# hpc4cmb/flacarray

Hardware: AMD Instinct MI355X
Metric: Msamples/s encode+decode, 4096ch x 1Msamp int32 (higher is better)
Workload: dtype int32

## Files before the change

### flacarray_amd/csrc/encode_fused.hpp

```cpp
#pragma once
#include "encode_kernels.hpp"
#include "quantize_kernels.hpp"

namespace fa {

constexpr int kFSmpWords = 65 * 32;
#ifndef FA_F_SCANW
#define FA_F_SCANW 4
#endif
#ifndef FA_F_RING
#define FA_F_RING 1024
#endif
constexpr int kFRingWords = FA_F_RING;
constexpr int kFRingMask = kFRingWords - 1;
constexpr int kFRingBlocks = kFRingWords / 64;
constexpr int kFRowBlocks = 12;
static_assert(kFRingBlocks - kFRowBlocks - 1 >= 1, "the ring must hold the longest row and a partial block beside what waits to be flushed");
constexpr int kFWaveWords = kFSmpWords + kFRingWords + 4 + 16;
constexpr int kFWaves = 4;
constexpr int kFCrcSlice = 1024;
constexpr int kFCrcXpow = 520;
#ifndef FA_F_SLEEP
#define FA_F_SLEEP 8
#endif
// ... 31 lines not shown
    const float* win;
    const uint4* hdr;
    uint8_t* blob;
    int64_t capacity;
    int64_t hb;
    uint32_t* frame_bytes;
    int64_t* frame_abs;
    FrameInfo* info;
    uint32_t* ticket;
    uint32_t* size_pub;
    unsigned long long* off_pub;
    int64_t* total;
    int* err;
    const uint16_t* crc_tab;
    unsigned long long* stamps;
    int64_t* starts;
    int64_t* nbytes;
};

__device__ __forceinline__ int fsmp_unit(int c1, int u) { return 32 * c1 + 4 * (u ^ (c1 & 7)); }
__device__ __forceinline__ int fsmp_idx(int s) {
    const int c1 = (s >> 5) + 1;
    return fsmp_unit(c1, (s >> 2) & 7) + (s & 3);
}

__device__ __forceinline__ int lane_id_opaque() {
    int l;
    asm volatile("v_mbcnt_lo_u32_b32 %0, -1, 0\n\tv_mbcnt_hi_u32_b32 %0, -1, %0" : "=v"(l));
    return l;
}
__device__ __forceinline__ int rice_fold(int r) { return (int)(((uint32_t)r << 1) ^ (uint32_t)(r >> 31)); }
__device__ __forceinline__ int dpp_wave_shr1(int old, int v) { return __builtin_amdgcn_update_dpp(old, v, 0x138, 0xF, 0xF, false); }

__device__ __forceinline__ uint16_t crc16_mulmod(uint16_t a, uint16_t b) {
    uint32_t r = 0;
#pragma unroll
    for (int i = 15; i >= 0; --i) {
        r = (r << 1) ^ ((r & 0x8000u) ? 0x18005u : 0u);
        if ((b >> i) & 1) r ^= a;
    }
    return (uint16_t)r;
}

template <typename T>
__device__ __forceinline__ T lb_load(const T* p) { return __hip_atomic_load(p, __ATOMIC_RELAXED, __HIP_MEMORY_SCOPE_AGENT); }

struct SplitRiceSearch {
    int pred_order, pmax, lane;
    uint32_t TA, TB, S, n, pb, SC, best;
    int M, p, k, bpo, kb;
    bool slot;
    __device__ __forceinline__ void start(uint32_t ta, uint32_t tb, int pred_order_, int pmax_, int lane_) {
        pred_order = pred_order_; pmax = pmax_; lane = lane_;
        TA = wave_incl_scan_u32(ta);
        TB = wave_incl_scan_u32(tb);
    }
    __device__ __forceinline__ void gather() {
        M = (2 << pmax) - 1;
        const int Lp = M - lane;
        slot = (Lp >= 1);
        const int po = slot ? (31 - __clz(Lp)) : 0;
        p = lane - (M + 1 - (2 << po));
        const uint32_t psz = 4096u >> po;
        const int cpp = 128 >> po;
        const bool inB = (po > 0) && (p >= (1 << (po - 1)));
        const int ph = inB ? (p - (1 << (po - 1))) : p;
        int hi_l = (po == 0) ? 63 : ((ph + 1) * cpp - 1);
        int lo_l = (po == 0) ? -1 : (ph * cpp - 1);
        hi_l &= 63;
        const int lo_c = lo_l < 0 ? 0 : (lo_l & 63);
        const uint32_t ah = (uint32_t)__builtin_amdgcn_ds_bpermute(hi_l << 2, (int)TA);
        const uint32_t bh = (uint32_t)__builtin_amdgcn_ds_bpermute(hi_l << 2, (int)TB);
        const uint32_t al = (uint32_t)__builtin_amdgcn_ds_bpermute(lo_c << 2, (int)TA);
        const uint32_t bl = (uint32_t)__builtin_amdgcn_ds_bpermute(lo_c << 2, (int)TB);
        uint32_t s;
        if (po == 0) s = ah + bh;
        else s = (inB ? bh : ah) - ((lo_l >= 0) ? (inB ? bl : al) : 0u);
        S = slot ? s : 0u;
        n = psz - ((p == 0) ? (uint32_t)pred_order : 0u);
        n = slot ? n : 1u;
    }
    __device__ __forceinline__ void params() {
        const uint32_t fpd = 0x40000u / n;
        const uint32_t m1 = S - 1;
        const uint32_t v = (__umulhi(m1, fpd) << 14) | ((m1 * fpd) >> 18);
        k = (S < 2 || v == 0) ? 0 : (32 - __clz((int)v));
        const uint32_t rest = (k != 0) ? (S >> ((k - 1) & 31)) : (S << 1);
        pb = 4u + (uint32_t)(1 + k) * n + rest - (n >> 1);
        pb = slot ? pb : 0u;
    }
    __device__ __forceinline__ void totals() {
        SC = wave_incl_scan_u32(pb);
        best = 0xffffffffu;
        bpo = 0;
        kb = 0;
    }
    __device__ __forceinline__ void order(int o) {
        const bool valid = (o <= pmax);
        const int base = valid ? (M + 1 - (2 << o)) : 0;
        const int end = valid ? (base + (1 << o) - 1) : 0;
        const uint32_t hi = (uint32_t)__builtin_amdgcn_readlane((int)SC, end);
        const uint32_t lo = (uint32_t)__builtin_amdgcn_readlane((int)SC, base > 0 ? base - 1 : 0);
        const uint32_t bits = hi - (base > 0 ? lo : 0u) + 6u;
        const int kg = __builtin_amdgcn_ds_bpermute(((base + lane) & 63) << 2, k);
        const bool take = valid && (bits < best);
        best = take ? bits : best;
        bpo = take ? o : bpo;
        kb = take ? kg : kb;
    }
};

__device__ __forceinline__ uint64_t split_rice_search_slow(uint64_t ta, uint64_t tb, int pred_order, int pmax, int lane, int* best_po,
                                                           int* kbest) {
    const uint64_t TA = wave_incl_scan_u64(ta), TB = wave_incl_scan_u64(tb);
    uint64_t best = 0;
    bool have = false;
// ... 59 lines not shown
                if ((uint32_t)lane < cnt) {
                    const uint64_t off = prefix + (incl - mine) + (uint64_t)(i / nf + 1u) * (uint64_t)a.hb;
                    __hip_atomic_store(a.off_pub + i, (unsigned long long)off, __ATOMIC_RELAXED, __HIP_MEMORY_SCOPE_AGENT);
#ifdef FA_TIMELINE
                    if (a.info) a.info[i].porder = (int32_t)(uint32_t)__builtin_amdgcn_s_memrealtime();
#endif
                }
                prefix += (uint32_t)__builtin_amdgcn_readlane((int)incl, 63);
                adv += cnt;
            }
            open = open && (cnt == 64u);
        }
        pos += adv;
        if (adv == 0) {
            __builtin_amdgcn_s_sleep(4);
            if (++idle > kLbSpinLimit) {
                if (lane == 0) atomicOr(a.err, 4);
                return;
            }
        } else {
            idle = 0;
        }
    }
    if (lane == 0) *a.total = (int64_t)(prefix + (uint64_t)a.n_stream * (uint64_t)a.hb);
}

#if defined(FA_UNIT_FUSED) || !defined(FA_SPLIT_UNITS)
template <int MLO, bool F32IN = false>
__global__ __launch_bounds__(256) __attribute__((amdgpu_waves_per_eu(MLO > 8 ? 2 : FA_F_WAVES, MLO > 8 ? 2 : FA_F_WAVES))) void encode_fused_kernel(FusedArgs a) {
    static_assert(MLO > 0, "levels 0-2 (fixed predictors, 1152-sample blocks) use the slot path");
    __shared__ __attribute__((aligned(16))) int32_t lds_all[kFWaves * kFWaveWords];
    __shared__ __attribute__((aligned(16))) uint16_t crc_s[kFCrcSlice];
    __shared__ uint32_t ticket_s;

    const int tid = threadIdx.x;
    const int lane = tid & 63;
    const int wave = __builtin_amdgcn_readfirstlane(tid >> 6);
    for (int i = tid; i < kFCrcSlice / 2; i += 256) reinterpret_cast<uint32_t*>(crc_s)[i] = reinterpret_cast<const uint32_t*>(a.crc_tab)[i];
    if (tid == 0) ticket_s = __hip_atomic_fetch_add(a.ticket, 1u, __ATOMIC_RELAXED, __HIP_MEMORY_SCOPE_AGENT);
    __syncthreads();
    const uint32_t ticket = (uint32_t)__builtin_amdgcn_readfirstlane((int)ticket_s);
    if (ticket == 0) {
        if (wave == 0) fused_scanner(a, lane);
        return;
    }
    const int64_t g = (int64_t)(ticket - 1) * kFWaves + wave;
    if (g >= a.total_frames) return;

    int32_t* smp = lds_all + wave * kFWaveWords;
    uint32_t* ring = reinterpret_cast<uint32_t*>(smp + kFSmpWords);
    uint8_t* kpar = reinterpret_cast<uint8_t*>(smp + kFSmpWords + kFRingWords + 4);
    uint32_t* scr = ring;

    const int64_t s = (int64_t)((uint32_t)g / (uint32_t)a.nframes);
    const int64_t f = g - s * a.nframes;
    if (f == a.nframes - 1 && a.tail_bs != kMaxBlock) return;
    constexpr int bs = kMaxBlock;
    const int32_t* src = a.data + (s * a.stream_size + f * (int64_t)bs);
    float q_off = 0.0f, q_gain = 0.0f;
    if constexpr (F32IN) { q_off = a.f_offsets[s]; q_gain = a.f_gains[s]; }
    auto load_row = [&](int j) __attribute__((always_inline)) {
        const int4 v = reinterpret_cast<const int4*>(src)[64 * j + lane];
        if constexpr (F32IN)
            return make_int4(quantise_f32(__int_as_float(v.x), q_off, q_gain), quantise_f32(__int_as_float(v.y), q_off, q_gain),
                             quantise_f32(__int_as_float(v.z), q_off, q_gain), quantise_f32(__int_as_float(v.w), q_off, q_gain));
        else
            return v;
    };
    const float* win = a.win;
    const uint4 fhe = a.hdr[f];
    const uint32_t fh_bits = 32u + ((fhe.w >> 8) & 0xFFu) + ((fhe.w >> 16) & 0xFFu) + (fhe.w >> 24) + 8u;

#define FA_IMAGE_ADDRS                                                                  \
    const int ln_ = lane_id_opaque();                                                   \
    const int K = fsmp_unit(ln_ + 1, 0);                                                \
    const int rowbase = fsmp_unit((ln_ >> 3) + 1, ln_ & 7);                             \
    const int hist7 = fsmp_unit(ln_, 7), hist6 = fsmp_unit(ln_, 6), hist5 = fsmp_unit(ln_, 5); \
    (void)K; (void)rowbase; (void)hist7; (void)hist6; (void)hist5
    constexpr int tailA7 = 32 * 64 + 4 * (7 ^ (64 & 7)), tailA6 = 32 * 64 + 4 * (6 ^ (64 & 7)), tailA5 = 32 * 64 + 4 * (5 ^ (64 & 7));

    FA_STAMP_INIT;
#ifdef FA_TIMELINE
    const uint32_t tl_start_ = (uint32_t)__builtin_amdgcn_s_memrealtime();
#endif
    int4 Bv[8];
    uint32_t orv = 0;
    int mn, mx;
    {
        FA_IMAGE_ADDRS;
        int4 hi[8], lo[8];
#pragma unroll
        for (int j = 0; j < 8; ++j) hi[j] = load_row(8 + j);
#pragma unroll
        for (int j = 0; j < 8; ++j) lo[j] = load_row(j);
        if (lane < 32) smp[lane] = 0;
        mn = hi[0].x;
        mx = hi[0].x;
#pragma unroll
        for (int j = 0; j < 8; ++j) {
            orv |= (uint32_t)(hi[j].x | hi[j].y | hi[j].z | hi[j].w);
            mn = min(min(mn, hi[j].x), hi[j].y);
            mn = min(min(mn, hi[j].z), hi[j].w);
            mx = max(max(mx, hi[j].x), hi[j].y);
            mx = max(max(mx, hi[j].z), hi[j].w);
            *reinterpret_cast<int4*>(&smp[rowbase + 256 * j]) = hi[j];
        }
#pragma unroll
        for (int t = 0; t < 8; ++t) Bv[t] = *reinterpret_cast<const int4*>(&smp[K ^ (4 * t)]);
#pragma unroll
        for (int j = 0; j < 8; ++j) {
            orv |= (uint32_t)(lo[j].x | lo[j].y | lo[j].z | lo[j].w);
            mn = min(min(mn, lo[j].x), lo[j].y);
            mn = min(min(mn, lo[j].z), lo[j].w);
            mx = max(max(mx, lo[j].x), lo[j].y);
            mx = max(max(mx, lo[j].z), lo[j].w);
            *reinterpret_cast<int4*>(&smp[rowbase + 256 * j]) = lo[j];
        }
    }
    mn = wave_min_i32(mn);
    mx = wave_max_i32(mx);
    const bool is_const = (mn == mx);
    orv = wave_or_u32(orv);
    const int wasted = orv ? (__ffs((int)orv) - 1) : 0;
    const int bps = 32 - wasted;
    if (__builtin_expect(wasted != 0, 0)) {
        FA_IMAGE_ADDRS;
#pragma unroll
        for (int t = 0; t < 8; ++t) {
            Bv[t].x >>= wasted; Bv[t].y >>= wasted; Bv[t].z >>= wasted; Bv[t].w >>= wasted;
            int4* p = reinterpret_cast<int4*>(&smp[K ^ (4 * t)]);
            int4 v = *p;
            v.x >>= wasted; v.y >>= wasted; v.z >>= wasted; v.w >>= wasted;
            *p = v;
        }
        mn >>= wasted;
        mx >>= wasted;
    }
    const bool narrow = (mn >= -(1 << 24)) && (mx < (1 << 24));
    lds_fence();

    FA_STAMP(0);
    const uint64_t verbatim_bits = 8 + (uint64_t)wasted + (uint64_t)bs * (uint64_t)bps;
    int type = 1;
    int order = 0, porder = 0, shift = 0, precision = 0;
    int kbest = 0;
    bool img_is_residual = false;
    bool win_small_l = false, win_small_f = false;
    int fo = -1;
    int32_t qkeep[MLO];
#pragma unroll
    for (int j = 0; j < MLO; ++j) qkeep[j] = 0;
    const int pmax_geo = a.pmax_full;
    auto pmax_for = [&](int pred_order) __attribute__((always_inline)) {
        int pm = pmax_geo;
        while (pm > 0 && (bs >> pm) <= pred_order) pm--;
        return pm;
    };

    auto hist_b = [&](const int4& own, const int4& tail) __attribute__((always_inline)) {
        int4 h;
        h.x = dpp_wave_shr1(tail.x, own.x);
        h.y = dpp_wave_shr1(tail.y, own.y);
        h.z = dpp_wave_shr1(tail.z, own.z);
        h.w = dpp_wave_shr1(tail.w, own.w);
        return h;
    };

    if (__builtin_expect(is_const, 0)) {
        type = 0;
    } else {
        uint64_t best_bits = verbatim_bits;
        double tot0 = 0.0, tot1 = 0.0, tot2 = 0.0, tot3 = 0.0, tot4 = 0.0;
        double mx0 = 0.0, mx1 = 0.0, mx2 = 0.0, mx3 = 0.0, mx4 = 0.0;
        uint64_t hA0 = 0, hA1 = 0, hA2 = 0, hA3 = 0, hA4 = 0;
        double dA0 = 0.0, dA1 = 0.0, dA2 = 0.0, dA3 = 0.0, dA4 = 0.0;
        if (__builtin_expect(narrow, 1)) {
            FA_IMAGE_ADDRS;
            const uint32_t BIAS = 0x80000000u;
            uint32_t s0 = 0, s1 = 0, s2 = 0, s3 = 0, s4 = 0;
            int p1, pe1, pe2, pe3;
            auto seed = [&](const int4& hh) __attribute__((always_inline)) {
                p1 = hh.w;
                pe1 = hh.w - hh.z;
                pe2 = pe1 - (hh.z - hh.y);
                pe3 = pe2 - ((hh.z - hh.y) - (hh.y - hh.x));
            };
            auto group = [&](auto mask_tag, const int4& xv, int gi0) __attribute__((always_inline)) {
                constexpr bool MASK = decltype(mask_tag)::value;
                const int xs[4] = {xv.x, xv.y, xv.z, xv.w};
#pragma unroll
                for (int e = 0; e < 4; ++e) {
                    const int x = xs[e];
                    const int e1 = x - p1, e2 = e1 - pe1, e3 = e2 - pe2;
                    const uint32_t xb = (uint32_t)x ^ BIAS;
                    const uint32_t n0 = sad_u32(xb, BIAS, s0);
                    const uint32_t n1 = sad_u32(xb, (uint32_t)p1 ^ BIAS, s1);
                    const uint32_t n2 = sad_u32((uint32_t)e1 ^ BIAS, (uint32_t)pe1 ^ BIAS, s2);
                    const uint32_t n3 = sad_u32((uint32_t)e2 ^ BIAS, (uint32_t)pe2 ^ BIAS, s3);
                    const uint32_t n4 = sad_u32((uint32_t)e3 ^ BIAS, (uint32_t)pe3 ^ BIAS, s4);
                    if constexpr (MASK) {
                        const int gi = gi0 + e;
                        s0 = n0;
                        s1 = (gi >= 1) ? n1 : s1;
                        s2 = (gi >= 2) ? n2 : s2;
                        s3 = (gi >= 3) ? n3 : s3;
                        s4 = (gi >= 4) ? n4 : s4;
                    } else {
                        s0 = n0; s1 = n1; s2 = n2; s3 = n3; s4 = n4;
                    }
                    p1 = x; pe1 = e1; pe2 = e2; pe3 = e3;
                }
            };
            uint64_t a0 = 0, a1 = 0, a2 = 0, a3 = 0, a4 = 0;
            auto fold = [&]() __attribute__((always_inline)) {
                a0 += s0; a1 += s1; a2 += s2; a3 += s3; a4 += s4;
                s0 = s1 = s2 = s3 = s4 = 0;
            };
            seed(*reinterpret_cast<const int4*>(&smp[hist7]));
            group(std::true_type{}, *reinterpret_cast<const int4*>(&smp[K]), 32 * lane);
#pragma unroll
            for (int t = 1; t < 4; ++t) group(std::false_type{}, *reinterpret_cast<const int4*>(&smp[K ^ (4 * t)]), 0);
            fold();
#pragma unroll
            for (int t = 4; t < 8; ++t) group(std::false_type{}, *reinterpret_cast<const int4*>(&smp[K ^ (4 * t)]), 0);
            fold();
            hA0 = a0; hA1 = a1; hA2 = a2; hA3 = a3; hA4 = a4;
            seed(hist_b(Bv[7], *reinterpret_cast<const int4*>(&smp[tailA7])));
#pragma unroll
            for (int t = 0; t < 4; ++t) group(std::false_type{}, Bv[t], 0);
            fold();
#pragma unroll
            for (int t = 4; t < 8; ++t) group(std::false_type{}, Bv[t], 0);
            fold();
            tot0 = (double)a0; tot1 = (double)a1; tot2 = (double)a2; tot3 = (double)a3; tot4 = (double)a4;
        } else {
            FA_IMAGE_ADDRS;
            double p1, pe1, pe2, pe3;
            auto seed = [&](const int4& h) __attribute__((always_inline)) {
                p1 = (double)h.w;
                pe1 = (double)h.w - (double)h.z;
                const double e1b = (double)h.z - (double)h.y;
                pe2 = pe1 - e1b;
                const double e2b = e1b - ((double)h.y - (double)h.x);
// ... 2 lines not shown
            auto group = [&](const int4& xv, int gi0) __attribute__((always_inline)) {
                const int xs[4] = {xv.x, xv.y, xv.z, xv.w};
#pragma unroll
                for (int e = 0; e < 4; ++e) {
                    const int gi = gi0 + e;
                    const double xd = (double)xs[e];
                    const double e1 = xd - p1;
                    const double e2 = e1 - pe1;
                    const double e3 = e2 - pe2;
                    const double e4 = e3 - pe3;
                    const double a0 = fa_fabs(xd);
                    const double a1 = (gi >= 1) ? fa_fabs(e1) : 0.0;
                    const double a2 = (gi >= 2) ? fa_fabs(e2) : 0.0;
                    const double a3 = (gi >= 3) ? fa_fabs(e3) : 0.0;
                    const double a4 = (gi >= 4) ? fa_fabs(e4) : 0.0;
                    tot0 += a0; tot1 += a1; tot2 += a2; tot3 += a3; tot4 += a4;
                    mx0 = __builtin_fmax(mx0, a0);
                    mx1 = __builtin_fmax(mx1, a1);
                    mx2 = __builtin_fmax(mx2, a2);
                    mx3 = __builtin_fmax(mx3, a3);
                    mx4 = __builtin_fmax(mx4, a4);
                    p1 = xd; pe1 = e1; pe2 = e2; pe3 = e3;
                }
            };
            seed(*reinterpret_cast<const int4*>(&smp[hist7]));
#pragma unroll 1
            for (int t = 0; t < 8; ++t) group(*reinterpret_cast<const int4*>(&smp[K ^ (4 * t)]), 32 * lane + 4 * t);
            dA0 = tot0; dA1 = tot1; dA2 = tot2; dA3 = tot3; dA4 = tot4;
            seed(hist_b(Bv[7], *reinterpret_cast<const int4*>(&smp[tailA7])));
#pragma unroll
            for (int t = 0; t < 8; ++t) group(Bv[t], 4096);
        }
        FA_STAMP(1);
        {
            double tsum[5] = {tot0, tot1, tot2, tot3, tot4};
            wave_sum_butterfly_n<5>(tsum);
            const double T0 = tsum[0], T1 = tsum[1], T2 = tsum[2], T3 = tsum[3], T4 = tsum[4];
            double M0 = 0.0, M1 = 0.0, M2 = 0.0, M3 = 0.0, M4 = 0.0;
            if (!narrow) {
                M0 = wave_max_f64(mx0); M1 = wave_max_f64(mx1); M2 = wave_max_f64(mx2); M3 = wave_max_f64(mx3);
                M4 = wave_max_f64(mx4);
            }
            const double lim = 2147483647.0;
            double smallest = 1.8446744073709552e19;
            if (M0 <= lim && T0 < smallest) { fo = 0; smallest = T0; }
            if (M1 <= lim && T1 < smallest) { fo = 1; smallest = T1; }
            if (M2 <= lim && T2 < smallest) { fo = 2; smallest = T2; }
            if (M3 <= lim && T3 < smallest) { fo = 3; smallest = T3; }
            if (M4 <= lim && T4 < smallest) { fo = 4; smallest = T4; }
        }
        uint64_t fixA, fixB;
        if (narrow) {
            const uint64_t tA = (fo == 0) ? hA0 : (fo == 1) ? hA1 : (fo == 2) ? hA2 : (fo == 3) ? hA3 : hA4;
            const double tt = (fo == 0) ? tot0 : (fo == 1) ? tot1 : (fo == 2) ? tot2 : (fo == 3) ? tot3 : tot4;
            fixA = tA;
            fixB = (uint64_t)tt - tA;
        } else {
            const double tA = (fo == 0) ? dA0 : (fo == 1) ? dA1 : (fo == 2) ? dA2 : (fo == 3) ? dA3 : dA4;
            const double tt = (fo == 0) ? tot0 : (fo == 1) ? tot1 : (fo == 2) ? tot2 : (fo == 3) ? tot3 : tot4;
            fixA = (uint64_t)tA;
            fixB = (uint64_t)(tt - tA);
        }
        int po_fix = 0, k_fix = 0;
        const int pmax_fix = pmax_for(fo < 0 ? 0 : fo);
        const bool small_fix = __all((fixA < (1u << 24)) && (fixB < (1u << 24)));
        win_small_f = small_fix;
        const bool fuse_search = fo >= 0 && pmax_fix <= 5 && a.max_lpc_order > 0 && small_fix;
        uint64_t est_fix = 0;
        auto apply_fixed = [&]() __attribute__((always_inline)) {
            if (est_fix < best_bits) {
                best_bits = est_fix;
                type = 2;
                order = fo;
                porder = po_fix;
                kbest = k_fix;
            }
        };
        if (__builtin_expect(fo >= 0 && !fuse_search, 0)) {
            uint64_t rb;
            if (pmax_fix <= 5 && small_fix) {
                SplitRiceSearch fs;
                fs.start((uint32_t)fixA, (uint32_t)fixB, fo, pmax_fix, lane);
                fs.gather(); fs.params(); fs.totals();
#pragma unroll
                for (int o = 5; o >= 0; --o) fs.order(o);
                po_fix = fs.bpo; k_fix = fs.kb; rb = fs.best;
            } else {
                rb = split_rice_search_slow(fixA, fixB, fo, pmax_fix, lane, &po_fix, &k_fix);
            }
            est_fix = 8 + (uint64_t)wasted + (uint64_t)fo * (uint64_t)bps + rb;
            apply_fixed();
        }

        FA_STAMP(2);
        int mlo = a.max_lpc_order;
        if (__builtin_expect(mlo > 0, 1)) {
            FA_IMAGE_ADDRS;
            double acc[MLO + 1];
#pragma unroll
            for (int j = 0; j <= MLO; ++j) acc[j] = 0.0;
            SplitRiceSearch fs;
            if (fuse_search) fs.start((uint32_t)fixA, (uint32_t)fixB, fo, pmax_fix, lane);
            double hist[MLO];
            struct WinV { double w[4]; };
            auto load_win = [&](int i0) __attribute__((always_inline)) {
                const float4 f = *reinterpret_cast<const float4*>(win + i0);
                WinV v;
                v.w[0] = (double)f.x; v.w[1] = (double)f.y; v.w[2] = (double)f.z; v.w[3] = (double)f.w;
                return v;
            };
            auto lag_group = [&](const int4& xv, const WinV& wv) __attribute__((always_inline)) {
                const int xs[4] = {xv.x, xv.y, xv.z, xv.w};
#pragma unroll
                for (int e = 0; e < 4; ++e) {
                    const double d = (double)xs[e] * wv.w[e];
                    acc[0] = __builtin_fma(d, d, acc[0]);
#pragma unroll
                    for (int j = 0; j < MLO; ++j) acc[j + 1] = __builtin_fma(d, hist[j], acc[j + 1]);
#pragma unroll
                    for (int j = MLO - 1; j > 0; --j) hist[j] = hist[j - 1];
                    hist[0] = d;
                }
            };
            auto search_stage = [&](int tt) __attribute__((always_inline)) {
                if (!fuse_search) return;
                if (tt == 1) fs.gather();
                if (tt == 3) fs.params();
                if (tt == 5) fs.totals();
                if (tt >= 7 && tt <= 12) fs.order(12 - tt);
            };
#if FA_F_PARK
            {
                int4* const pk = reinterpret_cast<int4*>(ring) + lane;
#pragma unroll
                for (int t = 0; t < 4; ++t) pk[64 * t] = Bv[4 + t];
// ... 24 lines not shown
            }
#if FA_F_PARK
            {
                uint32_t pin = 16u * (uint32_t)lane;
                asm volatile("" : "+v"(pin) : "v"(__double2loint(acc[MLO])));
                const int4* const pk = reinterpret_cast<const int4*>(reinterpret_cast<const char*>(ring) + pin);
#pragma unroll
                for (int t = 0; t < 4; ++t) Bv[4 + t] = pk[64 * t];
            }
#endif
            {
                const int g0 = 2048 + 32 * lane;
                const int4 h7 = hist_b(Bv[7], *reinterpret_cast<const int4*>(&smp[tailA7]));
                const int4 h6 = hist_b(Bv[6], *reinterpret_cast<const int4*>(&smp[tailA6]));
                int4 h5 = make_int4(0, 0, 0, 0);
                if constexpr (MLO > 8) h5 = hist_b(Bv[5], *reinterpret_cast<const int4*>(&smp[tailA5]));
                const int hs[12] = {h7.w, h7.z, h7.y, h7.x, h6.w, h6.z, h6.y, h6.x, h5.w, h5.z, h5.y, h5.x};
#pragma unroll
                for (int j = 0; j < MLO; ++j) hist[j] = (double)hs[j] * (double)win[g0 - 1 - j];
#pragma unroll
                for (int tb = 0; tb < 8; tb += FA_F_WBATCH) {
                    WinV wv[FA_F_WBATCH];
#pragma unroll
                    for (int t = 0; t < FA_F_WBATCH; ++t) wv[t] = load_win(g0 + 4 * (tb + t));
#pragma unroll
                    for (int t = 0; t < FA_F_WBATCH; ++t) {
                        lag_group(Bv[tb + t], wv[t]);
                        search_stage(8 + tb + t);
                    }
                    __builtin_amdgcn_sched_barrier(0);
                }
            }
            FA_STAMP(4);
            if (fuse_search) {
                po_fix = fs.bpo;
                k_fix = fs.kb;
                est_fix = 8 + (uint64_t)wasted + (uint64_t)fo * (uint64_t)bps + (uint64_t)fs.best;
                apply_fixed();
            }
            double autoc[MLO + 1];
#if FA_F_BFLY_N
#pragma unroll
            for (int j = 0; j <= MLO; ++j) autoc[j] = acc[j];
            wave_sum_butterfly_n<MLO + 1>(autoc);
#else
#pragma unroll
            for (int j = 0; j <= MLO; ++j) autoc[j] = wave_sum_butterfly(acc[j]);
#endif

            FA_STAMP(5);
            if (__builtin_expect(autoc[0] != 0.0, 1)) {
                float* coef = reinterpret_cast<float*>(scr);
                double* err = reinterpret_cast<double*>(scr + 160);
                int* meta = reinterpret_cast<int*>(scr + 220);
                if (lane == 0) meta[0] = levinson<MLO>(autoc, mlo, coef, err);
                lds_fence();
                const int usable = meta[0];
                int prec = a.precision;
                int lo;
                {
                    double mybits = 1e300;
                    if (lane < usable) {
                        const double e = err[lane];
                        const double error_scale = a.escale_full;
                        double bpsv;
                        if (e > 0.0) {
                            bpsv = 0.5 * det_log2(error_scale * e);
                            if (!(bpsv >= 0.0)) bpsv = 0.0;
                        } else if (e < 0.0) {
                            bpsv = 1e32;
                        } else {
                            bpsv = 0.0;
                        }
                        mybits = bpsv * (double)(bs - (lane + 1)) + (double)((lane + 1) * (bps + prec));
                    }
                    double bestb = 4294967295.0;
                    int bi = 0;
#pragma unroll
                    for (int o = 0; o < MLO; ++o) {
                        const double b = readlane_f64(mybits, o);
                        if (o < usable && b < bestb) { bestb = b; bi = o; }
                    }
                    lo = bi + 1;
                }
                if (bps <= 17) {
                    const int limp = 32 - bps - ilog2_u64((uint64_t)lo);
                    if (prec > limp) prec = limp;
                }
                int sh = 0;
                int32_t qreg[MLO];
#pragma unroll
                for (int j = 0; j < MLO; ++j) qreg[j] = 0;
                int ok = 0;
                if (prec >= 2) ok = (quantize_coefs_t<MLO>(coef + (lo - 1) * MLO, lo, prec, qreg, &sh) == 0) ? 1 : 0;
                ok = __builtin_amdgcn_readfirstlane(ok);
                sh = __builtin_amdgcn_readfirstlane(sh);
#pragma unroll
                for (int j = 0; j < MLO; ++j) qreg[j] = __builtin_amdgcn_readfirstlane(qreg[j]);
                FA_STAMP(6);
                if (__builtin_expect(ok != 0, 1)) {
                    FA_IMAGE_ADDRS;
                    const double scale = bitsd((uint64_t)(1023 - sh) << 52);
                    double qd[MLO];
#pragma unroll
                    for (int j = 0; j < MLO; ++j) qd[j] = (double)qreg[j] * scale;
                    double tlA = 0.0, tlB = 0.0;
                    double hx[MLO];
                    const int4 a7 = *reinterpret_cast<const int4*>(&smp[hist7]), a6 = *reinterpret_cast<const int4*>(&smp[hist6]);
                    const int4 a5 = *reinterpret_cast<const int4*>(&smp[hist5]);
                    const int4 b7 = hist_b(Bv[7], *reinterpret_cast<const int4*>(&smp[tailA7]));
                    const int4 b6 = hist_b(Bv[6], *reinterpret_cast<const int4*>(&smp[tailA6]));
                    int4 b5 = make_int4(0, 0, 0, 0);
                    if constexpr (MLO > 8) b5 = hist_b(Bv[5], *reinterpret_cast<const int4*>(&smp[tailA5]));
                    lds_fence();
                    auto fold_f64 = [&](double r) __attribute__((always_inline)) {
                        return (int)(uint32_t)__builtin_fabs(__builtin_fma(r, 2.0, 0.5));
                    };
                    auto res_group = [&](auto mask_tag, const int4& xv, int gi0, double& tl) __attribute__((always_inline)) {
                        constexpr bool MASK = decltype(mask_tag)::value;
                        const int xs[4] = {xv.x, xv.y, xv.z, xv.w};
                        int rs[4];
#pragma unroll
                        for (int e = 0; e < 4; ++e) {
                            const double xd = (double)xs[e];
#if FA_F_CEIL
                            double t = xd;
#pragma unroll
                            for (int j = 0; j < MLO; ++j) t = __builtin_fma(-qd[j], hx[j], t);
                            const double r = fa_ceil(t);
#else
                            double sum = 0.0;
#pragma unroll
// ... 5 lines not shown
                                const bool v = (gi0 + e >= lo);
                                tl += v ? fa_fabs(r) : 0.0;
                                rs[e] = v ? fold_f64(r) : xs[e];
                            } else {
                                tl += fa_fabs(r);
                                rs[e] = fold_f64(r);
                            }
#pragma unroll
                            for (int j = MLO - 1; j > 0; --j) hx[j] = hx[j - 1];
                            hx[0] = xd;
                        }
                        return make_int4(rs[0], rs[1], rs[2], rs[3]);
                    };
                    constexpr int kWarmGroups = (MLO + 3) / 4;
                    {
                        const int hs[12] = {a7.w, a7.z, a7.y, a7.x, a6.w, a6.z, a6.y, a6.x, a5.w, a5.z, a5.y, a5.x};
#pragma unroll
                        for (int j = 0; j < MLO; ++j) hx[j] = (double)hs[j];
#pragma unroll
                        for (int t = 0; t < 8; ++t) {
                            int4* px = reinterpret_cast<int4*>(&smp[K ^ (4 * t)]);
                            if (t < kWarmGroups) *px = res_group(std::true_type{}, *px, 32 * lane + 4 * t, tlA);
                            else *px = res_group(std::false_type{}, *px, 0, tlA);
                        }
                    }
                    {
                        const int hs[12] = {b7.w, b7.z, b7.y, b7.x, b6.w, b6.z, b6.y, b6.x, b5.w, b5.z, b5.y, b5.x};
#pragma unroll
                        for (int j = 0; j < MLO; ++j) hx[j] = (double)hs[j];
#pragma unroll
                        for (int t = 0; t < 8; ++t) Bv[t] = res_group(std::false_type{}, Bv[t], 0, tlB);
                    }
                    FA_STAMP(7);
                    img_is_residual = true;
                    const int pmax = pmax_for(lo);
                    int po_l = 0, k_l = 0;
                    uint64_t rbits;
                    const bool small_l = __all((tlA < 16777216.0) && (tlB < 16777216.0));
                    bool lpc_in_range = true;
                    if (__builtin_expect(!small_l, 0)) {
                        bool hit = false;
#pragma unroll 1
                        for (int t = 0; t < 8; ++t) {
                            const int4 ra = *reinterpret_cast<const int4*>(&smp[K ^ (4 * t)]);
                            const int ras[4] = {ra.x, ra.y, ra.z, ra.w};
#pragma unroll
                            for (int e = 0; e < 4; ++e) hit = hit || ((32 * lane + 4 * t + e >= lo) && (uint32_t)ras[e] == 0xffffffffu);
                        }
#pragma unroll
                        for (int t = 0; t < 8; ++t)
                            hit = hit || (uint32_t)Bv[t].x == 0xffffffffu || (uint32_t)Bv[t].y == 0xffffffffu || (uint32_t)Bv[t].z == 0xffffffffu ||
                                  (uint32_t)Bv[t].w == 0xffffffffu;
                        lpc_in_range = !__any(hit);
                    }
                    win_small_l = small_l;
                    if (pmax <= 5 && small_l) {
                        SplitRiceSearch ls;
                        ls.start((uint32_t)tlA, (uint32_t)tlB, lo, pmax, lane);
                        ls.gather(); ls.params(); ls.totals();
#pragma unroll
                        for (int o = 5; o >= 0; --o) ls.order(o);
                        po_l = ls.bpo; k_l = ls.kb; rbits = ls.best;
                    } else {
                        rbits = split_rice_search_slow((uint64_t)tlA, (uint64_t)tlB, lo, pmax, lane, &po_l, &k_l);
                    }
                    if (lpc_in_range) {
                        const uint64_t est = 8 + (uint64_t)wasted + 4 + 5 + (uint64_t)lo * (uint64_t)(prec + bps) + rbits;
                        if (est < best_bits) {
                            best_bits = est;
                            type = 3;
                            order = lo;
                            porder = po_l;
                            kbest = k_l;
                            shift = sh;
                            precision = prec;
#pragma unroll
                            for (int j = 0; j < MLO; ++j) qkeep[j] = qreg[j];
                        }
                    }
                }
                lds_fence();
            }
        }
    }

    FA_STAMP(8);
    const int lane_w = lane_id_opaque();
    auto reload_image = [&]() __attribute__((always_inline)) {
        FA_IMAGE_ADDRS;
#pragma unroll 1
        for (int half = 1; half >= 0; --half) {
#pragma unroll
            for (int j = 0; j < 8; ++j) {
                int4 v = load_row(8 * half + j);
                v.x >>= wasted; v.y >>= wasted; v.z >>= wasted; v.w >>= wasted;
                *reinterpret_cast<int4*>(&smp[rowbase + 256 * j]) = v;
            }
            if (half == 1) {
#pragma unroll
                for (int t = 0; t < 8; ++t) Bv[t] = *reinterpret_cast<const int4*>(&smp[K ^ (4 * t)]);
            }
        }
        lds_fence();
    };
    if (__builtin_expect(type == 2, 0)) {
        if (img_is_residual) {
            reload_image();
            img_is_residual = false;
        }
        {
            FA_IMAGE_ADDRS;
            const int4 ha = *reinterpret_cast<const int4*>(&smp[hist7]);
            const int4 hb2 = hist_b(Bv[7], *reinterpret_cast<const int4*>(&smp[tailA7]));
            lds_fence();
            int64_t x1, x2, x3, x4;
            auto fgroup = [&](const int4& xv, int gi0) __attribute__((always_inline)) {
                const int xs[4] = {xv.x, xv.y, xv.z, xv.w};
                int rs[4];
#pragma unroll
                for (int e = 0; e < 4; ++e) {
                    const int64_t x0 = xs[e];
                    int64_t r;
                    if (order == 0) r = x0;
                    else if (order == 1) r = x0 - x1;
                    else if (order == 2) r = x0 - 2 * x1 + x2;
                    else if (order == 3) r = x0 - 3 * x1 + 3 * x2 - x3;
                    else r = x0 - 4 * x1 + 6 * x2 - 4 * x3 + x4;
// ... 49 lines not shown
                else size_group(std::false_type{}, clamp_tag, rv, kA, 0, bitsA);
            }
#pragma unroll
            for (int t = 0; t < 8; ++t) size_group(std::false_type{}, clamp_tag, Bv[t], kB, 0, bitsB);
        };
        if (__builtin_expect((type == 3) ? win_small_l : win_small_f, 1)) size_lane(std::false_type{});
        else size_lane(std::true_type{});
        bitsA += (8 - kWarmGroupsS) * 4 * (kA + 1u);
        bitsB += 32u * (kB + 1u);
        if (((uint32_t)lane_w & (cpp - 1u)) == 0u || cpp > 64u) {
            if (cpp <= 64u) { bitsA += (uint32_t)plen; bitsB += (uint32_t)plen; }
            else if (lane_w == 0) bitsA += (uint32_t)plen;
        }
        uint32_t rA = bitsA, rB = bitsB;
        rA += (uint32_t)xchg_i32<0>((int)rA); rB += (uint32_t)xchg_i32<0>((int)rB);
        rA += (uint32_t)xchg_i32<1>((int)rA); rB += (uint32_t)xchg_i32<1>((int)rB);
        rA += (uint32_t)xchg_i32<2>((int)rA); rB += (uint32_t)xchg_i32<2>((int)rB);
        const bool row_over = __any((rA > (uint32_t)kRowCapBits) || (rB > (uint32_t)kRowCapBits));
        const uint64_t exact = 6 + wave_sum_u64((uint64_t)bitsA + bitsB) + 8 + (uint64_t)wasted + (uint64_t)order * (uint64_t)bps +
                               ((type == 3) ? (4 + 5 + (uint64_t)order * (uint64_t)precision) : 0);
        if (row_over || exact > verbatim_bits) {
            type = 1;
            order = 0;
            porder = 0;
        }
        sub_bits = (uint32_t)exact;
    }
    if (type == 0) sub_bits = 8u + (uint32_t)wasted + (uint32_t)bps;
    if (type == 1) sub_bits = (uint32_t)verbatim_bits;
    const uint32_t total_bytes = ((fh_bits + sub_bits + 7u) >> 3) + 2u;
    const uint32_t L = total_bytes - 2u;

    FA_STAMP(9);
    const uint32_t F = (uint32_t)a.total_frames;
    const uint32_t gu = (uint32_t)g;
#ifdef FA_TIMELINE
    if (lane_w == 0 && a.info) {
        a.info[g].wasted = (int32_t)tl_start_;
        a.info[g].shift = (int32_t)(uint32_t)__builtin_amdgcn_s_memrealtime();
        __builtin_amdgcn_s_waitcnt(0);
    }
#endif
    if (lane_w == 0) {
        __hip_atomic_store(a.size_pub + gu, 0x80000000u | total_bytes, __ATOMIC_RELAXED, __HIP_MEMORY_SCOPE_AGENT);
        a.frame_bytes[g] = total_bytes;
    }
    (void)F;
#ifndef FA_TIMELINE
    if (lane_w == 0 && a.info) {
        FrameInfo fi;
        fi.type = type;
        fi.order = (type >= 2) ? order : 0;
        fi.porder = (type >= 2) ? porder : 0;
        fi.wasted = wasted;
        fi.shift = (type == 3) ? shift : 0;
        fi.precision = (type == 3) ? precision : 0;
        fi.nbytes = (int32_t)total_bytes;
        fi.blocksize = bs;
        a.info[g] = fi;
    }
#endif

#ifdef FA_F_ANALYSIS_ONLY
    if (lane_w == 0) a.frame_abs[g] = g * (int64_t)kSlotBytes + (s + 1) * a.hb;
    return;
#endif
// ... 183 lines not shown
        else if (lane_w == 1) { fv = fhe.y; fnb = (fhe.w >> 8) & 0xFFu; }
        else if (lane_w == 2) { fv = fhe.z & 0xFFFFu; fnb = (fhe.w >> 16) & 0xFFu; }
        else if (lane_w == 3) { fv = fhe.z >> 16; fnb = fhe.w >> 24; }
        else if (lane_w == 4) { fv = ((fhe.w & 0xFFu) << 8) | (uint32_t)((tc << 1) | (wasted ? 1 : 0)); fnb = 16; }
        else if (lane_w == 5) { if (wasted) { fv = 1; fnb = (uint32_t)wasted; } }
        else if (lane_w < kL_lpc) {
            if (lane_w - kL_warm < nwarm) {
                fv = (uint32_t)smp[fsmp_idx(lane_w - kL_warm)] & smask;
                fnb = (uint32_t)bps;
            }
        }
        else if (lane_w == kL_lpc) { if (type == 3) { fv = ((uint32_t)(precision - 1) << 5) | (uint32_t)shift; fnb = 9; } }
        else if (lane_w < kL_rice) {
            if (type == 3 && lane_w - kL_coef < order) {
                int32_t q = 0;
#pragma unroll
                for (int j = 0; j < MLO; ++j) q = (lane_w - kL_coef == j) ? qkeep[j] : q;
                fv = (uint32_t)q & ((1u << precision) - 1u);
                fnb = (uint32_t)precision;
            }
        }
        else if (lane_w == kL_rice) { if (type >= 2) { fv = ((rice2 ? 1u : 0u) << 4) | (uint32_t)porder; fnb = 6; } }
        const uint32_t incl = wave_incl_scan_u32(fnb);
        if (fnb) put_bits(incl - fnb, fv, fnb);
        pos = (uint32_t)__builtin_amdgcn_readlane((int)incl, 63);
    }
    lds_fence();
    FA_STAMP(10);

    if (__builtin_expect(type == 1, 0)) {
        const uint32_t mask = (bps == 32) ? 0xffffffffu : ((1u << bps) - 1u);
#pragma unroll 1
        for (int j = 0; j < 16; ++j) {
            const int4 rv = load_row(j);
            const int rs[4] = {rv.x >> wasted, rv.y >> wasted, rv.z >> wasted, rv.w >> wasted};
            flush_blocks((uint32_t)(256 * bps), false);
            uint32_t p = pos + (uint32_t)(4 * bps) * (uint32_t)lane_w;
#pragma unroll
            for (int e = 0; e < 4; ++e) {
                put_bits(p, (uint32_t)rs[e] & mask, (uint32_t)bps);
                p += (uint32_t)bps;
            }
            pos += (uint32_t)(256 * bps);
        }
    } else if (type >= 2) {
        FA_IMAGE_ADDRS;
        const uint32_t ps = (uint32_t)(bs >> porder);
        const int l2ps = 12 - porder;
        auto store_b = [&]() __attribute__((always_inline)) {
#pragma unroll
            for (int t = 0; t < 8; ++t) *reinterpret_cast<int4*>(&smp[K ^ (4 * t)]) = Bv[t];
        };
        {
            const int cb = (ln_ >> 2) + 1;
            const int r8a = 32 * cb + 4 * ((2 * (ln_ & 3)) ^ (cb & 7)), r8b = 32 * cb + 4 * ((2 * (ln_ & 3) + 1) ^ (cb & 7));
            auto row8 = [&](auto first_tag, int j) __attribute__((always_inline)) {
                constexpr bool FIRST = decltype(first_tag)::value;
                const uint32_t gb = (uint32_t)(512 * j + 8 * lane_w);
                const int4 va = *reinterpret_cast<const int4*>(&smp[r8a + 512 * (j & 3)]);
                const int4 vb = *reinterpret_cast<const int4*>(&smp[r8b + 512 * (j & 3)]);
                const uint32_t us[8] = {(uint32_t)va.x, (uint32_t)va.y, (uint32_t)va.z, (uint32_t)va.w,
                                        (uint32_t)vb.x, (uint32_t)vb.y, (uint32_t)vb.z, (uint32_t)vb.w};
                const uint32_t pidx = gb >> l2ps;
                const uint32_t k = kpar[pidx], kp1 = k + 1u;
                const uint32_t pstart = (pidx == 0u) ? (uint32_t)order : (pidx << l2ps);
                const bool newp = FIRST ? (gb <= pstart && pstart < gb + 8u) : ((gb & (ps - 1u)) == 0u);
                uint32_t q[8];
// ... 241 lines not shown
```

### flacarray_amd/csrc/flac_math.hpp

```cpp
#pragma once
#include <stdint.h>

#if defined(__HIPCC__)
#define FA_HD __host__ __device__ __forceinline__
#else
#define FA_HD inline
#endif

#if defined(FA_UNIT_FUSED) || defined(FA_UNIT_PLACED)
#define FA_GLOBAL static
#else
#define FA_GLOBAL
#endif

namespace fa {

constexpr int kMaxBlock = 4096;
constexpr int kChunk = 64;
constexpr int kRow = 256;
constexpr int kRowCapBits = 12288;
constexpr int kRiceLimit = 31;
constexpr int kMaxLpcOrder = 12;
constexpr int kSlotBytes = 16640;

// ... 35 lines not shown
}

FA_HD double det_log2(double x) {
    uint64_t b = dbits(x);
    int e = (int)((b >> 52) & 0x7ff) - 1023;
    double m = bitsd((b & 0x000fffffffffffffULL) | 0x3ff0000000000000ULL);
    if (m > 1.4142135623730951) { m = m * 0.5; e += 1; }
    double s = (m - 1.0) / (m + 1.0);
    double z = s * s;
    double p = 1.0 / 21.0;
    p = p * z + 1.0 / 19.0;
    p = p * z + 1.0 / 17.0;
    p = p * z + 1.0 / 15.0;
    p = p * z + 1.0 / 13.0;
    p = p * z + 1.0 / 11.0;
    p = p * z + 1.0 / 9.0;
    p = p * z + 1.0 / 7.0;
    p = p * z + 1.0 / 5.0;
    p = p * z + 1.0 / 3.0;
    p = p * z + 1.0;
    return (double)e + (2.8853900817779268 * s) * p;
}

FA_HD double fa_floor(double x) {
#if defined(__HIP_DEVICE_COMPILE__)
    return __builtin_floor(x);
#else
    return __builtin_floor(x);
#endif
}
FA_HD double fa_ceil(double x) { return __builtin_ceil(x); }
FA_HD double fa_fabs(double x) { return __builtin_fabs(x); }

template <int MLO>
FA_HD int levinson(const double* autoc, int max_order, float* coef, double* err_out) {
    double lpc[MLO];
    double err = autoc[0];
#pragma unroll
    for (int i = 0; i < MLO; ++i) {
        if (i < max_order) {
            double r = -autoc[i + 1];
#pragma unroll
            for (int j = 0; j < MLO; ++j)
                if (j < i) r = r - lpc[j] * autoc[i - j];
            r = r / err;
            lpc[i] = r;
#pragma unroll
            for (int j = 0; j < MLO / 2; ++j) {
                if (j < (i >> 1)) {
                    double tmp = lpc[j];
                    lpc[j] = lpc[j] + r * lpc[i - 1 - j];
                    lpc[i - 1 - j] = lpc[i - 1 - j] + r * tmp;
                }
            }
            if (i & 1) lpc[i >> 1] = lpc[i >> 1] + lpc[i >> 1] * r;
            err = err * (1.0 - r * r);
#pragma unroll
            for (int j = 0; j < MLO; ++j)
                if (j <= i) coef[i * MLO + j] = (float)(-lpc[j]);
            err_out[i] = err;
            if (err == 0.0) return i + 1;
        }
    }
    return max_order;
}

FA_HD int best_lpc_order(const double* err, int max_order, int total_samples, int overhead_bits) {
    double error_scale = 0.5 / (double)total_samples;
    int best_index = 0;
    double best_bits = 4294967295.0;
    for (int indx = 0; indx < max_order; ++indx) {
        int order = indx + 1;
        double bps;
// ... 138 lines not shown
```

Baseline: 204,100.

## Table-driven Rice divisors, biased fixed residuals, full-order Levinson, and stop-after probes

Replaces the per-lane integer division 0x40000/n in the Rice parameter search with a constexpr table of reciprocals copied into LDS, or a shift for power-of-two partitions. Keeps the fixed-predictor residual state in pre-biased unsigned form so the XOR per SAD operand goes away. Specialises Levinson to compile without the order guard when the runtime max order equals the template order, and uses opaque lane ids in several places to influence register allocation. Also adds FA_F_STOP_AFTER early-exit probes for stage timing, which are compiled out by default.

```diff
diff --git a/flacarray_amd/csrc/encode_fused.hpp b/flacarray_amd/csrc/encode_fused.hpp
--- a/flacarray_amd/csrc/encode_fused.hpp
+++ b/flacarray_amd/csrc/encode_fused.hpp
@@ -87,6 +87,35 @@
 __device__ __forceinline__ int rice_fold(int r) { return (int)(((uint32_t)r << 1) ^ (uint32_t)(r >> 31)); }
 __device__ __forceinline__ int dpp_wave_shr1(int old, int v) { return __builtin_amdgcn_update_dpp(old, v, 0x138, 0xF, 0xF, false); }
 
+#ifdef FA_F_STOP_AFTER
+constexpr uint32_t kFStopBytes = 16;
+__device__ __forceinline__ void fa_sink1(uint32_t v) { asm volatile("" ::"v"(v)); }
+__device__ __forceinline__ void fa_sink1(int v) { fa_sink1((uint32_t)v); }
+__device__ __forceinline__ void fa_sink1(bool v) { fa_sink1((uint32_t)v); }
+__device__ __forceinline__ void fa_sink1(uint64_t v) { fa_sink1((uint32_t)v); fa_sink1((uint32_t)(v >> 32)); }
+__device__ __forceinline__ void fa_sink1(double v) { fa_sink1((uint32_t)__double2loint(v)); fa_sink1((uint32_t)__double2hiint(v)); }
+__device__ __forceinline__ void fa_sink1(const int4& v) { fa_sink1(v.x); fa_sink1(v.y); fa_sink1(v.z); fa_sink1(v.w); }
+template <typename T, int N>
+__device__ __forceinline__ void fa_sink1(const T (&v)[N]) {
+#pragma unroll
+    for (int i = 0; i < N; ++i) fa_sink1(v[i]);
+}
+template <typename... T>
+__device__ __forceinline__ void fa_sink(const T&... v) { (fa_sink1(v), ...); }
+#define FA_STOP(k, ...)                                                                              \
+    if constexpr ((k) == FA_F_STOP_AFTER) {                                                          \
+        fa_sink(__VA_ARGS__);                                                                        \
+        if (lane_id_opaque() == 0) {                                                                 \
+            __hip_atomic_store(a.size_pub + g, 0x80000000u | kFStopBytes, __ATOMIC_RELAXED, __HIP_MEMORY_SCOPE_AGENT); \
+            a.frame_bytes[g] = kFStopBytes;                                                          \
+            a.frame_abs[g] = g * (int64_t)kFStopBytes + (s + 1) * a.hb;                              \
+        }                                                                                            \
+        return;                                                                                      \
+    }
+#else
+#define FA_STOP(k, ...) do { } while (0)
+#endif
+
 __device__ __forceinline__ uint16_t crc16_mulmod(uint16_t a, uint16_t b) {
     uint32_t r = 0;
 #pragma unroll
@@ -100,13 +129,25 @@
 template <typename T>
 __device__ __forceinline__ T lb_load(const T* p) { return __hip_atomic_load(p, __ATOMIC_RELAXED, __HIP_MEMORY_SCOPE_AGENT); }
 
+constexpr int kFpdOrders = 13;
+constexpr int kFpdWords = 6 * kFpdOrders;
+struct FpdTable { uint32_t v[kFpdWords]; };
+constexpr FpdTable make_fpd_table() {
+    FpdTable t{};
+    for (int po = 0; po < 6; ++po)
+        for (int o = 0; o < kFpdOrders; ++o) t.v[kFpdOrders * po + o] = 0x40000u / ((4096u >> po) - (uint32_t)o);
+    return t;
+}
+__constant__ FpdTable kFpdP0 = make_fpd_table();
+
 struct SplitRiceSearch {
     int pred_order, pmax, lane;
-    uint32_t TA, TB, S, n, pb, SC, best;
+    const uint32_t* fpd_tab;
+    uint32_t TA, TB, S, n, fpd, pb, SC, best;
     int M, p, k, bpo, kb;
     bool slot;
-    __device__ __forceinline__ void start(uint32_t ta, uint32_t tb, int pred_order_, int pmax_, int lane_) {
-        pred_order = pred_order_; pmax = pmax_; lane = lane_;
+    __device__ __forceinline__ void start(uint32_t ta, uint32_t tb, int pred_order_, int pmax_, int lane_, const uint32_t* fpd_tab_) {
+        pred_order = pred_order_; pmax = pmax_; lane = lane_; fpd_tab = fpd_tab_;
         TA = wave_incl_scan_u32(ta);
         TB = wave_incl_scan_u32(tb);
     }
@@ -134,9 +175,10 @@
         S = slot ? s : 0u;
         n = psz - ((p == 0) ? (uint32_t)pred_order : 0u);
         n = slot ? n : 1u;
+        const uint32_t q0 = fpd_tab[kFpdOrders * po + pred_order];
+        fpd = !slot ? 0x40000u : (p == 0) ? q0 : (64u << po);
     }
     __device__ __forceinline__ void params() {
-        const uint32_t fpd = 0x40000u / n;
         const uint32_t m1 = S - 1;
         const uint32_t v = (__umulhi(m1, fpd) << 14) | ((m1 * fpd) >> 18);
         k = (S < 2 || v == 0) ? 0 : (32 - __clz((int)v));
@@ -262,11 +304,14 @@
     __shared__ __attribute__((aligned(16))) int32_t lds_all[kFWaves * kFWaveWords];
     __shared__ __attribute__((aligned(16))) uint16_t crc_s[kFCrcSlice];
     __shared__ uint32_t ticket_s;
+    __shared__ uint32_t fpd_s[kFpdWords];
+    static_assert(MLO < kFpdOrders, "kFpdP0 covers predictor orders up to 12");
 
     const int tid = threadIdx.x;
     const int lane = tid & 63;
     const int wave = __builtin_amdgcn_readfirstlane(tid >> 6);
     for (int i = tid; i < kFCrcSlice / 2; i += 256) reinterpret_cast<uint32_t*>(crc_s)[i] = reinterpret_cast<const uint32_t*>(a.crc_tab)[i];
+    if (tid < kFpdWords) fpd_s[tid] = kFpdP0.v[tid];
     if (tid == 0) ticket_s = __hip_atomic_fetch_add(a.ticket, 1u, __ATOMIC_RELAXED, __HIP_MEMORY_SCOPE_AGENT);
     __syncthreads();
     const uint32_t ticket = (uint32_t)__builtin_amdgcn_readfirstlane((int)ticket_s);
@@ -289,8 +334,8 @@
     const int32_t* src = a.data + (s * a.stream_size + f * (int64_t)bs);
     float q_off = 0.0f, q_gain = 0.0f;
     if constexpr (F32IN) { q_off = a.f_offsets[s]; q_gain = a.f_gains[s]; }
-    auto load_row = [&](int j) __attribute__((always_inline)) {
-        const int4 v = reinterpret_cast<const int4*>(src)[64 * j + lane];
+    auto load_row = [&](int j, int ln) __attribute__((always_inline)) {
+        const int4 v = reinterpret_cast<const int4*>(src)[64 * j + ln];
         if constexpr (F32IN)
             return make_int4(quantise_f32(__int_as_float(v.x), q_off, q_gain), quantise_f32(__int_as_float(v.y), q_off, q_gain),
                              quantise_f32(__int_as_float(v.z), q_off, q_gain), quantise_f32(__int_as_float(v.w), q_off, q_gain));
@@ -320,9 +365,9 @@
         FA_IMAGE_ADDRS;
         int4 hi[8], lo[8];
 #pragma unroll
-        for (int j = 0; j < 8; ++j) hi[j] = load_row(8 + j);
-#pragma unroll
-        for (int j = 0; j < 8; ++j) lo[j] = load_row(j);
+        for (int j = 0; j < 8; ++j) hi[j] = load_row(8 + j, lane);
+#pragma unroll
+        for (int j = 0; j < 8; ++j) lo[j] = load_row(j, lane);
         if (lane < 32) smp[lane] = 0;
         mn = hi[0].x;
         mx = hi[0].x;
@@ -370,6 +415,7 @@
     lds_fence();
 
     FA_STAMP(0);
+    FA_STOP(0, Bv, mn, mx, wasted, narrow);
     const uint64_t verbatim_bits = 8 + (uint64_t)wasted + (uint64_t)bs * (uint64_t)bps;
     int type = 1;
     int order = 0, porder = 0, shift = 0, precision = 0;
@@ -408,12 +454,14 @@
             FA_IMAGE_ADDRS;
             const uint32_t BIAS = 0x80000000u;
             uint32_t s0 = 0, s1 = 0, s2 = 0, s3 = 0, s4 = 0;
-            int p1, pe1, pe2, pe3;
+            int p1, pe1, pe2;
+            uint32_t p1b, pe1b, pe2b, pe3b;
             auto seed = [&](const int4& hh) __attribute__((always_inline)) {
                 p1 = hh.w;
                 pe1 = hh.w - hh.z;
                 pe2 = pe1 - (hh.z - hh.y);
-                pe3 = pe2 - ((hh.z - hh.y) - (hh.y - hh.x));
+                const int pe3 = pe2 - ((hh.z - hh.y) - (hh.y - hh.x));
+                p1b = (uint32_t)p1 ^ BIAS; pe1b = (uint32_t)pe1 ^ BIAS; pe2b = (uint32_t)pe2 ^ BIAS; pe3b = (uint32_t)pe3 ^ BIAS;
             };
             auto group = [&](auto mask_tag, const int4& xv, int gi0) __attribute__((always_inline)) {
                 constexpr bool MASK = decltype(mask_tag)::value;
@@ -421,13 +469,14 @@
 #pragma unroll
                 for (int e = 0; e < 4; ++e) {
                     const int x = xs[e];
-                    const int e1 = x - p1, e2 = e1 - pe1, e3 = e2 - pe2;
                     const uint32_t xb = (uint32_t)x ^ BIAS;
+                    const int e1 = x - p1, e2 = e1 - pe1;
+                    const uint32_t e1b = xb - (uint32_t)p1, e2b = e1b - (uint32_t)pe1, e3b = e2b - (uint32_t)pe2;
                     const uint32_t n0 = sad_u32(xb, BIAS, s0);
-                    const uint32_t n1 = sad_u32(xb, (uint32_t)p1 ^ BIAS, s1);
-                    const uint32_t n2 = sad_u32((uint32_t)e1 ^ BIAS, (uint32_t)pe1 ^ BIAS, s2);
-                    const uint32_t n3 = sad_u32((uint32_t)e2 ^ BIAS, (uint32_t)pe2 ^ BIAS, s3);
-                    const uint32_t n4 = sad_u32((uint32_t)e3 ^ BIAS, (uint32_t)pe3 ^ BIAS, s4);
+                    const uint32_t n1 = sad_u32(xb, p1b, s1);
+                    const uint32_t n2 = sad_u32(e1b, pe1b, s2);
+                    const uint32_t n3 = sad_u32(e2b, pe2b, s3);
+                    const uint32_t n4 = sad_u32(e3b, pe3b, s4);
                     if constexpr (MASK) {
                         const int gi = gi0 + e;
                         s0 = n0;
@@ -438,7 +487,8 @@
                     } else {
                         s0 = n0; s1 = n1; s2 = n2; s3 = n3; s4 = n4;
                     }
-                    p1 = x; pe1 = e1; pe2 = e2; pe3 = e3;
+                    p1 = x; pe1 = e1; pe2 = e2;
+                    p1b = xb; pe1b = e1b; pe2b = e2b; pe3b = e3b;
                 }
             };
             uint64_t a0 = 0, a1 = 0, a2 = 0, a3 = 0, a4 = 0;
@@ -507,6 +557,7 @@
             for (int t = 0; t < 8; ++t) group(Bv[t], 4096);
         }
         FA_STAMP(1);
+        FA_STOP(1, Bv, tot0, tot1, tot2, tot3, tot4, hA0, hA1, hA2, hA3, hA4, mx0, mx1, mx2, mx3, mx4, dA0, dA1, dA2, dA3, dA4);
         {
             double tsum[5] = {tot0, tot1, tot2, tot3, tot4};
             wave_sum_butterfly_n<5>(tsum);
@@ -555,7 +606,7 @@
             uint64_t rb;
             if (pmax_fix <= 5 && small_fix) {
                 SplitRiceSearch fs;
-                fs.start((uint32_t)fixA, (uint32_t)fixB, fo, pmax_fix, lane);
+                fs.start((uint32_t)fixA, (uint32_t)fixB, fo, pmax_fix, lane, fpd_s);
                 fs.gather(); fs.params(); fs.totals();
 #pragma unroll
                 for (int o = 5; o >= 0; --o) fs.order(o);
@@ -568,6 +619,7 @@
         }
 
         FA_STAMP(2);
+        FA_STOP(2, Bv, fo, fixA, fixB, fuse_search, best_bits, type, po_fix, k_fix);
         int mlo = a.max_lpc_order;
         if (__builtin_expect(mlo > 0, 1)) {
             FA_IMAGE_ADDRS;
@@ -575,7 +627,7 @@
 #pragma unroll
             for (int j = 0; j <= MLO; ++j) acc[j] = 0.0;
             SplitRiceSearch fs;
-            if (fuse_search) fs.start((uint32_t)fixA, (uint32_t)fixB, fo, pmax_fix, lane);
+            if (fuse_search) fs.start((uint32_t)fixA, (uint32_t)fixB, fo, pmax_fix, lane, fpd_s);
             double hist[MLO];
             struct WinV { double w[4]; };
             auto load_win = [&](int i0) __attribute__((always_inline)) {
@@ -666,6 +718,7 @@
                 }
             }
             FA_STAMP(4);
+            FA_STOP(4, Bv, acc, fs.best, fs.bpo, fs.kb, best_bits);
             if (fuse_search) {
                 po_fix = fs.bpo;
                 k_fix = fs.kb;
@@ -683,19 +736,21 @@
 #endif
 
             FA_STAMP(5);
+            FA_STOP(5, Bv, autoc, best_bits, type, porder, kbest);
             if (__builtin_expect(autoc[0] != 0.0, 1)) {
                 float* coef = reinterpret_cast<float*>(scr);
                 double* err = reinterpret_cast<double*>(scr + 160);
                 int* meta = reinterpret_cast<int*>(scr + 220);
-                if (lane == 0) meta[0] = levinson<MLO>(autoc, mlo, coef, err);
+                const int ln = lane_id_opaque();
+                if (ln == 0) meta[0] = (mlo == MLO) ? levinson<MLO, true>(autoc, MLO, coef, err) : levinson<MLO>(autoc, mlo, coef, err);
                 lds_fence();
                 const int usable = meta[0];
                 int prec = a.precision;
                 int lo;
                 {
                     double mybits = 1e300;
-                    if (lane < usable) {
-                        const double e = err[lane];
+                    if (ln < usable) {
+                        const double e = err[ln];
                         const double error_scale = a.escale_full;
                         double bpsv;
                         if (e > 0.0) {
@@ -706,7 +761,7 @@
                         } else {
                             bpsv = 0.0;
                         }
-                        mybits = bpsv * (double)(bs - (lane + 1)) + (double)((lane + 1) * (bps + prec));
+                        mybits = bpsv * (double)(bs - (ln + 1)) + (double)((ln + 1) * (bps + prec));
                     }
                     double bestb = 4294967295.0;
                     int bi = 0;
@@ -732,6 +787,7 @@
 #pragma unroll
                 for (int j = 0; j < MLO; ++j) qreg[j] = __builtin_amdgcn_readfirstlane(qreg[j]);
                 FA_STAMP(6);
+                FA_STOP(6, Bv, qreg, sh, ok, lo, prec, best_bits, type, porder, kbest);
                 if (__builtin_expect(ok != 0, 1)) {
                     FA_IMAGE_ADDRS;
                     const double scale = bitsd((uint64_t)(1023 - sh) << 52);
@@ -803,6 +859,7 @@
                         for (int t = 0; t < 8; ++t) Bv[t] = res_group(std::false_type{}, Bv[t], 0, tlB);
                     }
                     FA_STAMP(7);
+                    FA_STOP(7, Bv, tlA, tlB, best_bits, type, porder, kbest);
                     img_is_residual = true;
                     const int pmax = pmax_for(lo);
                     int po_l = 0, k_l = 0;
@@ -816,7 +873,7 @@
                             const int4 ra = *reinterpret_cast<const int4*>(&smp[K ^ (4 * t)]);
                             const int ras[4] = {ra.x, ra.y, ra.z, ra.w};
 #pragma unroll
-                            for (int e = 0; e < 4; ++e) hit = hit || ((32 * lane + 4 * t + e >= lo) && (uint32_t)ras[e] == 0xffffffffu);
+                            for (int e = 0; e < 4; ++e) hit = hit || ((32 * ln_ + 4 * t + e >= lo) && (uint32_t)ras[e] == 0xffffffffu);
                         }
 #pragma unroll
                         for (int t = 0; t < 8; ++t)
@@ -827,13 +884,13 @@
                     win_small_l = small_l;
                     if (pmax <= 5 && small_l) {
                         SplitRiceSearch ls;
-                        ls.start((uint32_t)tlA, (uint32_t)tlB, lo, pmax, lane);
+                        ls.start((uint32_t)tlA, (uint32_t)tlB, lo, pmax, lane_id_opaque(), fpd_s);
                         ls.gather(); ls.params(); ls.totals();
 #pragma unroll
                         for (int o = 5; o >= 0; --o) ls.order(o);
                         po_l = ls.bpo; k_l = ls.kb; rbits = ls.best;
                     } else {
-                        rbits = split_rice_search_slow((uint64_t)tlA, (uint64_t)tlB, lo, pmax, lane, &po_l, &k_l);
+                        rbits = split_rice_search_slow((uint64_t)tlA, (uint64_t)tlB, lo, pmax, lane_id_opaque(), &po_l, &k_l);
                     }
                     if (lpc_in_range) {
                         const uint64_t est = 8 + (uint64_t)wasted + 4 + 5 + (uint64_t)lo * (uint64_t)(prec + bps) + rbits;
@@ -856,6 +913,7 @@
     }
 
     FA_STAMP(8);
+    FA_STOP(8, Bv, type, order, porder, kbest, shift, precision, qkeep);
     const int lane_w = lane_id_opaque();
     auto reload_image = [&]() __attribute__((always_inline)) {
         FA_IMAGE_ADDRS;
@@ -863,7 +921,7 @@
         for (int half = 1; half >= 0; --half) {
 #pragma unroll
             for (int j = 0; j < 8; ++j) {
-                int4 v = load_row(8 * half + j);
+                int4 v = load_row(8 * half + j, ln_);
                 v.x >>= wasted; v.y >>= wasted; v.z >>= wasted; v.w >>= wasted;
                 *reinterpret_cast<int4*>(&smp[rowbase + 256 * j]) = v;
             }
@@ -979,6 +1037,7 @@
     const uint32_t L = total_bytes - 2u;
 
     FA_STAMP(9);
+    FA_STOP(9, Bv, total_bytes, type, order, porder, kbest, shift, precision, qkeep, plen);
     const uint32_t F = (uint32_t)a.total_frames;
     const uint32_t gu = (uint32_t)g;
 #ifdef FA_TIMELINE
@@ -1228,7 +1287,7 @@
         const uint32_t mask = (bps == 32) ? 0xffffffffu : ((1u << bps) - 1u);
 #pragma unroll 1
         for (int j = 0; j < 16; ++j) {
-            const int4 rv = load_row(j);
+            const int4 rv = load_row(j, lane_w);
             const int rs[4] = {rv.x >> wasted, rv.y >> wasted, rv.z >> wasted, rv.w >> wasted};
             flush_blocks((uint32_t)(256 * bps), false);
             uint32_t p = pos + (uint32_t)(4 * bps) * (uint32_t)lane_w;
diff --git a/flacarray_amd/csrc/flac_math.hpp b/flacarray_amd/csrc/flac_math.hpp
--- a/flacarray_amd/csrc/flac_math.hpp
+++ b/flacarray_amd/csrc/flac_math.hpp
@@ -91,13 +91,13 @@
 FA_HD double fa_ceil(double x) { return __builtin_ceil(x); }
 FA_HD double fa_fabs(double x) { return __builtin_fabs(x); }
 
-template <int MLO>
+template <int MLO, bool FULL = false>
 FA_HD int levinson(const double* autoc, int max_order, float* coef, double* err_out) {
     double lpc[MLO];
     double err = autoc[0];
 #pragma unroll
     for (int i = 0; i < MLO; ++i) {
-        if (i < max_order) {
+        if (FULL || i < max_order) {
             double r = -autoc[i + 1];
 #pragma unroll
             for (int j = 0; j < MLO; ++j)
```

New measurement: 209,100 (median of 6 runs). +2.4%, better.
